# sfu-compbio/scalce

Hardware: AMD Instinct MI355X
Metric: input FASTQ MB/s compressed, 100 bp reads, bit-exact decompress (higher is better)
Workload: dtype u8

## Files before the change

scalce_amd/csrc/host_entropy.inc:

```
struct AcJob {
  scalce_batch *b;
  int m;
  const u8 *sym;
  u64 nsym;
  u32 nblk;
  bool general;
  u32 max_total = 0;
};
static const u64 AC_STRIDE = (u64)AC_BLOCK_SYMS + 4096;
constexpr u32 AC_LOG_WORDS = 1024;

static int ac_prepare(AcJob &j, hipStream_t s, bool framed_output = true, bool full_stride = false, bool allow_in_place = false) {
  scalce_batch *b = j.b;
  scalce_ctx *c = b->ctx;
  const int m = j.m;
  u32 *table = b->table[m].as<u32>();
  ENSURE(b, b->ac_tab[m], sizeof(uint4) * 512000);
  ENSURE(b, b->ac_cum[m], sizeof(u32) * 6400 * 81);
  BatchScratch::TableInfo *tinfo = &b->d_scr->tinfo[m];
  HIP_TRY(c, hipMemsetAsync(tinfo, 0, sizeof *tinfo, s));
  ENSURE(b, b->ac_tab8[m], sizeof(u64) * (6400 * 81 + 2));
  LAUNCH(ac_table_k, cdiv(6400, 64), 64, 0, s, table, b->ac_tab[m].as<uint4>(), b->ac_cum[m].as<u32>(), reinterpret_cast<u32 *>(&tinfo->max_total), b->ac_tab8[m].as<u64>(),
         tinfo->cost);
  BatchScratch::TableInfo th = {0, {0, 0}};
  { int rc = read_words(b, tinfo, &th, sizeof th / 4, s); if (rc) return rc; }
  const u32 max_total = (u32)th.max_total;
  j.general = max_total > (1u << 30) || getenv("SCALCE_AC_GENERAL") != nullptr;
  j.max_total = max_total;
  j.nblk = (u32)cdiv(j.nsym, AC_BLOCK_SYMS);
  {
    u64 stride = AC_STRIDE;
    const char *scale_env = getenv("SCALCE_AC_STRIDE_SCALE");
    const bool full = scale_env && atof(scale_env) == 0.0;
    if (!full && !full_stride && th.cost[1]) {
      double bytes_per_symbol = (double)th.cost[0] / 256.0 / 8.0 / (double)th.cost[1];
      if (scale_env) bytes_per_symbol *= atof(scale_env);
      const u64 est = (u64)((double)AC_BLOCK_SYMS * bytes_per_symbol * 1.08) + 65536;
      stride = std::min<u64>(AC_STRIDE, (est + 15) & ~15ull);
    }
    b->ac_stride[m] = stride;
  }
  b->in_place_now[m] = allow_in_place && b->code_in_place && !b->in_place_suspended && !b->qs_in_ws && j.nblk &&
                       j.sym == b->qs(m).as<u8>() && b->qs(m).cap >= j.nsym + 64 + AC_INPLACE_PAD;
  if (b->in_place_now[m]) {
    b->ac_stride[m] = AC_BLOCK_SYMS;
    b->ac_base[m] = b->qs(m).as<u8>();
    ENSURE(b, b->ac_log[m], sizeof(u32) * AC_LOG_WORDS * (size_t)j.nblk + 64);
  } else {
    ENSURE(b, b->ac_blocks[m], (size_t)j.nblk * b->ac_stride[m] + 4096 + 64);
    b->ac_base[m] = b->ac_blocks[m].as<u8>();
  }
  ENSURE(b, b->ac_sizes[m], sizeof(u32) * (j.nblk + 2));
  ENSURE(b, b->ac_off[m], sizeof(u64) * (j.nblk + 2));
  if (framed_output && !b->frame_on_demand) ENSURE(b, b->out_qual[m], (size_t)j.nblk * (b->ac_stride[m] + 4) + 64);
  ENSURE(b, b->ac_scan, sizeof(u64) * (scan_ws_elems(j.nblk ? j.nblk : 1) + 64));
  if (!j.nblk) b->out_qual_bytes[m] = 0;
  return SCALCE_OK;
}

enum AcLaunchKind { AC_SINGLE, AC_PAIRED, AC_RECODE, AC_WINDOW, AC_GROUP, AC_GROUP_LAST };
struct AcShape {
  int blocks_per_wg;
  u32 lanes;
};

static int ac_blocks_override() {
  const char *e = getenv("SCALCE_AC_BLOCKS_PER_WG");
  const int v = e ? atoi(e) : 0;
  return (v == 4 || v == 8 || v == 64) ? v : 0;
}

static u32 ac_lanes_override() {
  const char *e = getenv("SCALCE_AC_LANES_USED");
  if (!e) return 0;
  const int v = atoi(e);
  return (u32)(v < 1 || v > 64 ? 32 : v);
}

static AcShape ac_shape(AcLaunchKind kind, u32 blocks, bool general, int device) {
  const int over = ac_blocks_override();
  int bpw;
  switch (kind) {
    case AC_SINGLE: bpw = over ? over : 1; break;
    case AC_PAIRED:
    case AC_RECODE: bpw = blocks <= 1024 ? 4 : 8; break;
    case AC_WINDOW: bpw = 8; break;
    default:
      bpw = blocks < 900 ? 4 : (kind == AC_GROUP_LAST && blocks <= 2048) ? 8 : 64;
      if (over) bpw = over;
  }
  if (bpw == 64 && general) bpw = 8;
  u32 lanes = ac_lanes_override();
  if (!lanes && kind == AC_GROUP_LAST && bpw == 64) {
    static int n_cus = 0;
    if (!n_cus) { hipDeviceProp_t pr; n_cus = hipGetDeviceProperties(&pr, device) == hipSuccess && pr.multiProcessorCount > 0 ? pr.multiProcessorCount : 256; }
    lanes = std::min<u32>(std::max<u32>(cdiv(blocks, (u32)n_cus), 8u), 64u);
  }
  return AcShape{bpw, lanes ? lanes : 32u};
}

static int ac_launch(AcJob *jobs, int njobs, AcLaunchKind kind, hipStream_t s, hipStream_t ps) {
  scalce_batch *lead = jobs[0].b;
  scalce_ctx *c = lead->ctx;
  u32 total = 0;
  bool general = false;
  for (int i = 0; i < njobs; i++) {
    total += jobs[i].nblk;
    general |= jobs[i].general;
    if (jobs[i].max_total > (1u << 29)) general = true;
  }
  if (!total) return SCALCE_OK;
  const AcShape shape = ac_shape(kind, total, general, c->device);
  AcEncArgs a;
  memset(&a, 0, sizeof a);
  a.slow_threshold = 32;
  a.chain_prio = 3u;
  a.helper_prio = 0u;
  a.test_poison = getenv("SCALCE_AC_TEST_POISON") ? (u32)atoi(getenv("SCALCE_AC_TEST_POISON")) : 0u;
  a.inplace_shift = getenv("SCALCE_AC_INPLACE_TEST") ? 2u : 0u;
  a.simd_load = c->d_simd_load.as<u32>();
  if (const char *e = getenv("SCALCE_AC_SLOW_THRESHOLD")) a.slow_threshold = (u32)atoi(e);
  auto join = [&]() -> int {
    if (ps == s) return SCALCE_OK;
    hipEvent_t ev = lead->ev_group;
    if (!ev) { HIP_TRY(c, hipEventCreateWithFlags(&ev, hipEventDisableTiming)); lead->ev_group = ev; }
    HIP_TRY(c, hipEventRecord(ev, ps));
    HIP_TRY(c, hipStreamWaitEvent(s, ev, 0));
    return SCALCE_OK;
  };
  hipEvent_t ke0 = nullptr, ke1 = nullptr;
  if (lead->ktiming) {
    if (lead->kev_used == lead->kev.size()) {
      hipEvent_t x, y;
      HIP_TRY(c, hipEventCreate(&x));
      HIP_TRY(c, hipEventCreate(&y));
      lead->kev.emplace_back(x, y);
    }
    ke0 = lead->kev[lead->kev_used].first; ke1 = lead->kev[lead->kev_used].second;
    lead->kev_used++;
  }
  if (shape.blocks_per_wg == 1) {
    if (njobs != 1) { set_err(c, "internal: ac_encode_k takes one job"); return SCALCE_ERR_ARG; }
    scalce_batch *b = jobs[0].b;
    const int m = jobs[0].m;
    a.sym = jobs[0].sym; a.nsym = jobs[0].nsym; a.tab = b->ac_tab[m].as<uint4>(); a.out = b->ac_base[m];
    a.out_stride = b->ac_stride[m]; a.out_cap = (u32)b->ac_stride[m]; a.out_size = b->ac_sizes[m].as<u32>(); a.err = b->d_err;
    { int rc = join(); if (rc) return rc; }
    if (ke0) hipEventRecord(ke0, s);
    if (general) LAUNCH(ac_encode_k<true>, total, 128, 0, s, a);
    else LAUNCH(ac_encode_k<false>, total, 128, 0, s, a);
    if (ke1) hipEventRecord(ke1, s);
  } else {
    if (total > lead->ac_desc_cap) {
      if (lead->ac_desc_host) hipHostFree(lead->ac_desc_host);
      lead->ac_desc_host = nullptr;
      lead->ac_desc_cap = 0;
      const u32 cap = std::max<u32>(total + total / 2, 8192u);
      HIP_TRY(c, hipHostMalloc(reinterpret_cast<void **>(&lead->ac_desc_host), sizeof(AcBlockDesc) * (size_t)cap, hipHostMallocDefault));
      lead->ac_desc_cap = cap;
    }
    const bool lanes = shape.blocks_per_wg == 64;
    AcBlockDesc *d = lead->ac_desc_host;
    u32 nd = 0;
    for (int i = 0; i < njobs; i++) {
      scalce_batch *b = jobs[i].b;
      const int m = jobs[i].m;
      for (u32 k = 0; k < jobs[i].nblk; k++) {
        AcBlockDesc x;
        const u64 off = (u64)k * AC_BLOCK_SYMS;
        x.sym = jobs[i].sym + off;
        x.tab = lanes ? reinterpret_cast<const uint4 *>(b->ac_tab8[m].as<u64>()) : b->ac_tab[m].as<uint4>();
        x.dst = reinterpret_cast<u32 *>(b->ac_base[m] + (u64)k * b->ac_stride[m]);
        x.cap = (u32)b->ac_stride[m];
        x.flags = 0; x.log = nullptr; x.log_cap = 0; x.pad_ = 0;
        if (b->in_place_now[m]) {
          const u64 left = jobs[i].nsym - (u64)k * AC_BLOCK_SYMS;
          if (left < AC_BLOCK_SYMS) x.cap = (u32)std::min<u64>(AC_BLOCK_SYMS, (left + AC_INPLACE_PAD) & ~3ull);
          x.flags = AC_BLOCK_IN_PLACE;
          x.log = b->ac_log[m].as<u32>() + (size_t)k * AC_LOG_WORDS;
          x.log_cap = AC_LOG_WORDS;
        }
        x.out_size = b->ac_sizes[m].as<u32>() + k;
        x.err = b->d_err;
        x.n = (u32)std::min<u64>(AC_BLOCK_SYMS, jobs[i].nsym - off);
        x.index = k;
        d[nd++] = x;
      }
    }
    ENSURE(lead, lead->ac_desc, sizeof(AcBlockDesc) * (size_t)lead->ac_desc_cap);
    HIP_TRY(c, hipMemcpyAsync(lead->ac_desc.p, d, sizeof(AcBlockDesc) * total, hipMemcpyHostToDevice, ps));
    a.desc = lead->ac_desc.as<AcBlockDesc>();
    a.nblocks = total;
    a.out_cap = (u32)AC_STRIDE;
    { int rc = join(); if (rc) return rc; }
    if (ke0) hipEventRecord(ke0, s);
    if (lanes) {
      a.lanes_used = shape.lanes;
      if (a.lanes_used <= 48) LAUNCH((ac_encode_lanes_k<true, 1, 48, 5>), cdiv(total, a.lanes_used), 256, 0, s, a);
      else LAUNCH((ac_encode_lanes_k<true, 1, 64, 5>), cdiv(total, a.lanes_used), 256, 0, s, a);
    } else if (shape.blocks_per_wg == 8) {
      if (general) LAUNCH((ac_encode_rows_k<true, 8>), cdiv(total, 8), 320, 0, s, a);
      else LAUNCH((ac_encode_rows_k<false, 8>), cdiv(total, 8), 320, 0, s, a);
    } else {
      if (general) LAUNCH((ac_encode_rows_k<true, 16>), cdiv(total, 4), 192, 0, s, a);
      else LAUNCH((ac_encode_rows_k<false, 16>), cdiv(total, 4), 192, 0, s, a);
    }
    if (ke1) hipEventRecord(ke1, s);
  }
  for (int i = 0; i < njobs; i++) {
    lead->k_in_bytes += jobs[i].nsym;
    jobs[i].b->ac_last_sym[jobs[i].m] = jobs[i].sym;
    jobs[i].b->ac_last_nsym[jobs[i].m] = jobs[i].nsym;
  }
  return SCALCE_OK;
}

static int ac_frame(AcJob &j, hipStream_t s) {
  scalce_batch *b = j.b;
  const int m = j.m;
  b->frame_virtual[m] = 0;
  if (!j.nblk) return SCALCE_OK;
  exclusive_scan<u64>(AcFrameLen{b->ac_sizes[m].as<u32>()}, j.nblk, StoreTo<u64>{b->ac_off[m].as<u64>()}, b->ac_scan.as<u64>(),
                      &b->d_scr->frame_bytes[m], s);
  if (b->frame_on_demand) {
    b->frame_virtual[m] = j.nblk;
    b->ent_pending[m] = j.nblk;
    return SCALCE_OK;
  }
  if (b->out_qual[m].cap < (size_t)j.nblk * (b->ac_stride[m] + 4) + 64) {
    u64 total = 0;
    { int rc = read_u64(b, &b->d_scr->frame_bytes[m], &total, 1, s); if (rc) return rc; }
    if (b->out_qual[m].cap < total + 64) ENSURE(b, b->out_qual[m], (size_t)(total + total / 16) + (32u << 20));
  }
  LAUNCH(ac_frame_k, dim3(cdiv(b->ac_stride[m], 16 * 256), j.nblk), 256, 0, s, b->ac_base[m], b->ac_stride[m],
         b->ac_sizes[m].as<u32>(), b->ac_off[m].as<u64>(), b->out_qual[m].as<u8>());
  b->ent_pending[m] = j.nblk;
  return SCALCE_OK;
}

static int encode_stream(scalce_batch *b, int m, const u8 *d_sym, u64 nsym, hipStream_t s) {
  AcJob j{b, m, d_sym, nsym, 0, false};
  int rc = ac_prepare(j, s);
  if (rc) return rc;
  if ((rc = ac_launch(&j, 1, AC_SINGLE, s, s))) return rc;
  return ac_frame(j, s);
}

static int entropy_recode_full(scalce_batch *b, hipStream_t s) {
  std::vector<AcJob> jobs;
  for (int m = 0; m < b->nm; m++) {
    if (!b->ac_last_sym[m] || !b->ac_last_nsym[m]) continue;
    AcJob j{b, m, b->ac_last_sym[m], b->ac_last_nsym[m], 0, false};
    int rc = ac_prepare(j, s, false, true);
    if (rc) return rc;
    jobs.push_back(j);
  }
  if (jobs.empty()) return SCALCE_OK;
  int rc = ac_launch(jobs.data(), (int)jobs.size(), AC_RECODE, s, s);
  if (rc) return rc;
  for (auto &j : jobs) { b->frame_deferred[j.m] = j.nblk; b->ent_pending[j.m] = 0; }
  return SCALCE_OK;
}

static int entropy_rerun_from_text(scalce_batch *b, hipStream_t s) {
  scalce_ctx *c = b->ctx;
  if (b->appending || b->base != 0 || !b->piece_text[0] || (b->nm == 2 && !b->piece_text[1])) {
    set_err(c, "a block coded in place outgrew its input and the shard's text is not at hand to run it again (scalce_batch_set_code_in_place)");
    return SCALCE_ERR_CAPACITY;
  }
  static const bool dbg = getenv("SCALCE_TRACE") != nullptr;
  if (dbg) fprintf(stderr, "scalce: batch %p: a block coded in place caught up with its input: the shard is run again from its text\n", (void *)b);
  const u8 *t1 = b->piece_text[0], *t2 = b->ntext == 2 ? b->piece_text[1] : nullptr;
  const u64 n1 = b->text_bytes[0], n2 = b->ntext == 2 ? b->text_bytes[1] : 0;
  for (int m = 0; m < 2; m++) { b->frame_deferred[m] = 0; b->ent_pending[m] = 0; b->in_place_now[m] = false; }
  b->in_place_suspended = true;
  b->reruns++;
  int rc = scalce_batch_front(b, t1, n1, t2, n2, s);
  if (!rc) rc = scalce_batch_entropy(b, nullptr, s);
  b->in_place_suspended = false;
  return rc;
}

static int entropy_collect(scalce_batch *b, hipStream_t s) {
  {
    bool open = false, tight = false, in_place = false;
    for (int m = 0; m < b->nm; m++) {
      open |= b->frame_deferred[m] != 0 || b->ent_pending[m] != 0;
      tight |= b->ac_stride[m] != 0 && b->ac_stride[m] < AC_STRIDE;
      in_place |= b->in_place_now[m];
    }
    if (open && tight) {
      DevErr e;
      HIP_TRY(b->ctx, hipMemcpyAsync(&e, b->d_err, sizeof e, hipMemcpyDeviceToHost, s));
      HIP_TRY(b->ctx, hipStreamSynchronize(s));
      if (e.code == E_ACOVERFLOW) {
        if (getenv("SCALCE_TRACE"))
          fprintf(stderr, "scalce: batch %p: block %llu outgrew its %llu-byte buffer (it needed %u): coding the shard again at the full stride\n",
                  (void *)b, (unsigned long long)e.where, (unsigned long long)b->ac_stride[0], e.aux);
        HIP_TRY(b->ctx, hipMemsetAsync(b->d_err, 0, sizeof(DevErr), s));
        if (in_place) return entropy_rerun_from_text(b, s);
        int rc = entropy_recode_full(b, s);
        if (rc) return rc;
      }
    }
  }
  for (int m = 0; m < b->nm; m++) {
    if (b->frame_deferred[m]) {
      AcJob j{b, m, nullptr, 0, b->frame_deferred[m], false};
      b->frame_deferred[m] = 0;
      int rc = ac_frame(j, s);
      if (rc) return rc;
    }
    if (!b->ent_pending[m]) continue;
    u64 total = 0;
    if (b->frame_virtual[m]) {
      b->frame_off_host[m].resize(b->frame_virtual[m]);
      HIP_TRY(b->ctx, hipMemcpyAsync(b->frame_off_host[m].data(), b->ac_off[m].p, sizeof(u64) * b->frame_virtual[m], hipMemcpyDeviceToHost, s));
    }
    { int rc = read_u64(b, &b->d_scr->frame_bytes[m], &total, 1, s); if (rc) return rc; }
    b->out_qual_bytes[m] = total;
    b->k_out_bytes += total - 4ull * b->ent_pending[m];
    b->ent_pending[m] = 0;
  }
  return SCALCE_OK;
}

static int ac_table_for(scalce_batch *b, int m, const uint32_t *d_table_override, u64 nsym, hipStream_t s) {
  scalce_ctx *c = b->ctx;
  u32 *table = b->table[m].as<u32>();
  if (d_table_override) {
    HIP_TRY(c, hipMemcpyAsync(table, d_table_override + (size_t)m * 512000, sizeof(u32) * 512000, hipMemcpyDeviceToDevice, s));
  } else {
    const u32 factor = 1 + (u32)(nsym / 0xFFFFFFFFull);
    LAUNCH(ac_scale_k, cdiv(512000, 256), 256, 0, s, b->freq4[m].as<u64>(), factor, table);
  }
  return SCALCE_OK;
}

constexpr u32 AC_WINDOW_BLOCKS = 2048;
static int entropy_windowed(scalce_batch *b, const uint32_t *d_table_override, hipStream_t s) {
  scalce_ctx *c = b->ctx;
  const u64 N = b->N;
  u32 W = AC_WINDOW_BLOCKS / (u32)b->nm;
  if (const char *e = getenv("SCALCE_AC_WINDOW_BLOCKS")) W = (u32)std::max(1, atoi(e));
  u64 used[2] = {0, 0}, nsym[2] = {0, 0};
  u32 nblk[2] = {0, 0}, most = 0;
  for (int m = 0; m < b->nm; m++) {
    nsym[m] = N * (u64)b->L[m];
    nblk[m] = cdiv(nsym[m], AC_BLOCK_SYMS);
    most = nblk[m] > most ? nblk[m] : most;
    b->frame_virtual[m] = 0;
    b->frame_off_host[m].clear();
    int rc = ac_table_for(b, m, d_table_override, nsym[m], s);
    if (rc) return rc;
    b->out_qual_bytes[m] = 0;
  }
  bool first = true;
  for (u32 w0 = 0; w0 < most; w0 += W) {
    AcJob jobs[2];
    int nj = 0;
    for (int m = 0; m < b->nm; m++) {
      if (w0 >= nblk[m]) continue;
      const u64 off = (u64)w0 * AC_BLOCK_SYMS;
      const u64 n = std::min<u64>(nsym[m] - off, (u64)W * AC_BLOCK_SYMS);
      jobs[nj] = AcJob{b, m, b->qs(m).as<u8>() + off, n, 0, false};
      int rc = ac_prepare(jobs[nj], s, false, true);
      if (rc) return rc;
      nj++;
    }
    if (!nj) break;
    int rc = ac_launch(jobs, nj, AC_WINDOW, s, s);
    if (rc) return rc;
    for (int i = 0; i < nj; i++) {
      const int m = jobs[i].m;
      exclusive_scan<u64>(AcFrameLen{b->ac_sizes[m].as<u32>()}, jobs[i].nblk, StoreTo<u64>{b->ac_off[m].as<u64>()}, b->ac_scan.as<u64>(),
                          &b->d_scr->frame_bytes[m], s);
      u64 total = 0;
      if ((rc = read_u64(b, &b->d_scr->frame_bytes[m], &total, 1, s))) return rc;
      if (first) {
        const u64 est = (u64)((double)total / (double)jobs[i].nsym * 1.03 * (double)nsym[m]) + (64u << 20);
        ENSURE(b, b->out_qual[m], est);
      }
      if ((rc = ensure_keep(b, b->out_qual[m], used[m] + total + 64, used[m], s))) return rc;
      LAUNCH(ac_frame_k, dim3(cdiv(b->ac_stride[m], 16 * 256), jobs[i].nblk), 256, 0, s, b->ac_base[m], b->ac_stride[m],
             b->ac_sizes[m].as<u32>(), b->ac_off[m].as<u64>(), b->out_qual[m].as<u8>() + used[m]);
      used[m] += total;
      b->k_out_bytes += total - 4ull * jobs[i].nblk;
    }
    first = false;
  }
  HIP_TRY(c, hipStreamSynchronize(s));
  for (int m = 0; m < b->nm; m++) { b->out_qual_bytes[m] = used[m]; b->ent_pending[m] = 0; }
  return SCALCE_OK;
}

extern "C" int scalce_batch_entropy_begin(scalce_batch *b, const uint32_t *d_table_override, void *stream) {
  if (!b) return SCALCE_ERR_ARG;
  hipStream_t s = (hipStream_t)stream;
  scalce_ctx *c = b->ctx;
  HIP_TRY(c, hipSetDevice(c->device));
  if (b->nq) {
    for (int m = 0; m < b->nm; m++) b->out_qual_bytes[m] = 0;
    return SCALCE_OK;
  }
  const u64 N = b->N;
  if (!b->p.no_ac) {
    u64 blocks = 0;
    for (int m = 0; m < b->nm; m++) blocks += cdiv(N * (u64)b->L[m], AC_BLOCK_SYMS);
    if (blocks > AC_WINDOW_BLOCKS || getenv("SCALCE_AC_WINDOW_BLOCKS")) return entropy_windowed(b, d_table_override, s);
  }
  if (b->nm == 2 && !b->p.no_ac && !ac_blocks_override()) {
    AcJob jobs[2];
    for (int m = 0; m < 2; m++) {
      const u64 nsym = N * (u64)b->L[m];
      int rc = ac_table_for(b, m, d_table_override, nsym, s);
      if (rc) return rc;
      jobs[m] = AcJob{b, m, b->qs(m).as<u8>(), nsym, 0, false};
      if ((rc = ac_prepare(jobs[m], s))) return rc;
    }
    int rc = ac_launch(jobs, 2, AC_PAIRED, s, s);
    if (rc) return rc;
    for (int m = 0; m < 2; m++)
      if ((rc = ac_frame(jobs[m], s))) return rc;
    return SCALCE_OK;
  }
  for (int m = 0; m < b->nm; m++) {
    const u64 nsym = N * (u64)b->L[m];
    if (b->p.no_ac) {
      b->out_qual_bytes[m] = nsym;
      continue;
    }
    int rc = ac_table_for(b, m, d_table_override, nsym, s);
    if (rc) return rc;
    if ((rc = encode_stream(b, m, b->qs(m).as<u8>(), nsym, s))) return rc;
  }
  return SCALCE_OK;
}

extern "C" int scalce_batch_entropy_begin_group(scalce_batch **bs, int n, void *prep_stream, void *stream) {
  return scalce_batch_entropy_begin_group_last(bs, n, prep_stream, stream, 0);
}
extern "C" int scalce_batch_entropy_begin_group_last(scalce_batch **bs, int n, void *prep_stream, void *stream, int last) {
  if (!bs || n <= 0 || n > SCALCE_GROUP_MAX || (last != 0 && last != 1)) return SCALCE_ERR_ARG;
  for (int i = 0; i < n; i++) if (!bs[i] || bs[i]->ctx != bs[0]->ctx) return SCALCE_ERR_ARG;
  hipStream_t ps = (hipStream_t)prep_stream, s = (hipStream_t)stream;
  scalce_ctx *c = bs[0]->ctx;
  HIP_TRY(c, hipSetDevice(c->device));
  std::vector<AcJob> jobs;
  for (int i = 0; i < n; i++) {
    scalce_batch *b = bs[i];
    for (int m = 0; m < b->nm; m++) {
      const u64 own = b->N * (u64)b->L[m];
      if (b->nq) { b->out_qual_bytes[m] = 0; continue; }
      if (b->p.no_ac) { b->out_qual_bytes[m] = own; continue; }
      AcJob j{b, m, b->ent_external[m] ? b->ent_sym[m] : b->qs(m).as<u8>(), b->ent_external[m] ? b->ent_nsym[m] : own, 0, false};
      if (!b->ent_external[m]) { int rc = ac_table_for(b, m, nullptr, own, ps); if (rc) return rc; }
      b->ent_external[m] = false;
      int rc = ac_prepare(j, ps, false, false, true);
      if (rc) return rc;
      jobs.push_back(j);
    }
  }
  if (jobs.empty()) return SCALCE_OK;
  int rc = ac_launch(jobs.data(), (int)jobs.size(), last ? AC_GROUP_LAST : AC_GROUP, s, ps);
  if (rc) return rc;
  for (auto &j : jobs) j.b->frame_deferred[j.m] = j.nblk;
  return SCALCE_OK;
}

extern "C" int scalce_batch_entropy_stream_prepare(scalce_batch *b, int mate, const uint32_t *d_table, const uint8_t *d_symbols,
                                                   uint64_t nsym, void *stream) {
  if (!b || mate < 0 || mate >= b->nm || !d_table || (nsym && !d_symbols) || b->p.no_ac || b->nq) return SCALCE_ERR_ARG;
  scalce_ctx *c = b->ctx;
  HIP_TRY(c, hipSetDevice(c->device));
  HIP_TRY(c, hipMemcpyAsync(b->table[mate].p, d_table, sizeof(u32) * 512000, hipMemcpyDeviceToDevice, (hipStream_t)stream));
  b->ent_sym[mate] = d_symbols;
  b->ent_nsym[mate] = nsym;
  b->ent_external[mate] = true;
  return SCALCE_OK;
}

extern "C" int scalce_batch_entropy_end(scalce_batch *b, void *stream) {
  if (!b) return SCALCE_ERR_ARG;
  HIP_TRY(b->ctx, hipSetDevice(b->ctx->device));
  return entropy_collect(b, (hipStream_t)stream);
}

extern "C" int scalce_batch_entropy(scalce_batch *b, const uint32_t *d_table_override, void *stream) {
  if (!b) return SCALCE_ERR_ARG;
  if (b->nq) return scalce_batch_entropy_begin(b, d_table_override, stream);
  StageTimer tm(b, ST_ENTROPY, (hipStream_t)stream);
  int rc = scalce_batch_entropy_begin(b, d_table_override, stream);
  if (rc) return rc;
  return entropy_collect(b, (hipStream_t)stream);
}

extern "C" int scalce_batch_entropy_stream_begin(scalce_batch *b, int mate, const uint32_t *d_table, const uint8_t *d_symbols,
                                                 uint64_t nsym, void *stream) {
  if (!b || mate < 0 || mate >= b->nm || !d_table || (nsym && !d_symbols) || b->p.no_ac || b->nq) return SCALCE_ERR_ARG;
  hipStream_t s = (hipStream_t)stream;
  scalce_ctx *c = b->ctx;
  HIP_TRY(c, hipSetDevice(c->device));
  HIP_TRY(c, hipMemcpyAsync(b->table[mate].p, d_table, sizeof(u32) * 512000, hipMemcpyDeviceToDevice, s));
  return encode_stream(b, mate, d_symbols, nsym, s);
}
extern "C" int scalce_batch_entropy_stream(scalce_batch *b, int mate, const uint32_t *d_table, const uint8_t *d_symbols,
                                           uint64_t nsym, void *stream) {
  if (!b) return SCALCE_ERR_ARG;
  StageTimer tm(b, ST_ENTROPY, (hipStream_t)stream);
  int rc = scalce_batch_entropy_stream_begin(b, mate, d_table, d_symbols, nsym, stream);
  if (rc) return rc;
  return entropy_collect(b, (hipStream_t)stream);
}

extern "C" int scalce_ac_scale(scalce_ctx *c, const uint64_t *d_counters, uint32_t factor, uint32_t *d_table, void *stream) {
  if (!c || !d_counters || !d_table || !factor) return SCALCE_ERR_ARG;
  HIP_TRY(c, hipSetDevice(c->device));
  LAUNCH(ac_scale_k, cdiv(512000, 256), 256, 0, (hipStream_t)stream, reinterpret_cast<const u64 *>(d_counters), factor, d_table);
  return SCALCE_OK;
}

extern "C" int scalce_copy_pieces(scalce_ctx *c, const uint8_t *d_src, uint8_t *d_dst, const uint64_t *d_piece_src,
                                  const uint64_t *d_piece_dst, uint32_t npieces, uint64_t total_bytes, void *stream) {
  if (!c) return SCALCE_ERR_ARG;
  if (!npieces || !total_bytes) return SCALCE_OK;
  HIP_TRY(c, hipSetDevice(c->device));
  LAUNCH(copy_pieces_k, cdiv(total_bytes + 15, 256 * 16 * CP_CHUNKS), 256, 0, (hipStream_t)stream, d_src, d_dst,
         reinterpret_cast<const u64 *>(d_piece_src), reinterpret_cast<const u64 *>(d_piece_dst), npieces, (u64)total_bytes);
  return SCALCE_OK;
}
```

scalce_amd/csrc/kernels_acl.hpp:

```cpp
#pragma once
#include "kernels_ac.hpp"

namespace scalce {

constexpr int ACL_STEPS = 16;

__device__ __forceinline__ void acl_step_general(u32 &lo, u32 &hi, const uint4 g, u32 &B, u32 &t) {
  const u32 R = hi - lo;
  u32 M;
  const bool wrap = __builtin_add_overflow(R, 1u, &M);
  const u32 qa = mulfrac_m(M, wrap, g.z, g.w);
  const u32 qb = mulfrac_m(M, wrap, g.x, g.y);
  const u32 nhi = (g.w == 0xFFFFFFFFu) ? hi : lo + qa - 1;
  const u32 nlo = lo + qb;
  B = qb;
  const u32 x = nlo ^ nhi;
  const u32 kf = x ? (u32)__clz(x) : 31u;
  const u32 ks = kf < 31u ? kf : 31u;
  const u32 z = ((nlo & ~nhi) << ks) << 1;
  const u32 u = (u32)__clz(~z);
  t = ks + u;
  lo = (nlo << t) & 0x7FFFFFFFu;
  hi = (nhi << t) | ((1u << t) - 1) | 0x80000000u;
}

__device__ __forceinline__ void acl_step_plain(u32 &lo, u32 &M, const uint4 g, u32 ones, u32 zero, u32 &B, u32 &t) {
  const u32 A1 = (u32)(((u64)M * g.w + (((u64)ones << 32) | __umulhi(M, g.z))) >> 32);
  B = (u32)(((u64)M * g.y + (((u64)zero << 32) | __umulhi(M, g.x))) >> 32);
  const u32 D = A1 - B;
  const u32 nlo = lo + B;
  t = renorm_count(nlo, D);
  M = (D + 1) << t;
  lo = nlo << t;
}

template <int LW, int SETS> struct AclRing { static constexpr int WORDS = 64; };
template <int LW>
struct AclSink {
  SCALCE_GLOBAL u32 *dst;
  u32 wcap;
  SCALCE_GLOBAL u32 *logtop;
  u32 logcap;
  u32 w2, w1, w0;
  u32 Qb;
  u32 ncar;
  u32 nlog;
  bool over;
  __device__ __forceinline__ void init(SCALCE_GLOBAL u32 *d, u32 cap_words, SCALCE_GLOBAL u32 *log, u32 log_words, u32 s0, u32 s1) {
    dst = d; wcap = cap_words;
    logtop = log ? log + (log_words - 1u) : d + (cap_words - 1u);
    logcap = log ? log_words : 0u;
    w2 = 0; w1 = (s0 << 24) | (s1 << 16); w0 = 0;
    Qb = 16; ncar = ~0u; nlog = 0; over = false;
  }
  __device__ __forceinline__ u32 final_words() const {
    const u32 wq = Qb >> 5;
    return wq ? wq - 1u : 0u;
  }
  __device__ __forceinline__ bool room() {
    if ((Qb >> 5) + 2 * ACL_STEPS + 2 + (logcap ? 0u : nlog) >= wcap) over = true;
    if (logcap && nlog + ACL_STEPS + 2 >= logcap) over = true;
    return !over;
  }
  __device__ __forceinline__ void step(u32 B, u32 Qa, u32 &val, u32 &wq) {
    const u32 pos = Qb & 31u;
    const u32 b_hi = B >> pos;
    const u32 b_lo = __builtin_amdgcn_alignbit(B, 0u, pos);
    u32 c0, c1;
    w0 = __builtin_addc(w0, b_lo, 0u, &c0);
    w1 = __builtin_addc(w1, b_hi, c0, &c1);
    w2 += c1;
    ncar = w2 < ncar ? w2 : ncar;
    wq = Qb >> 5;
    val = w2;
    const bool f = (Qa >> 5) != wq;
    w2 = f ? w1 : w2;
    w1 = f ? w0 : w1;
    w0 = f ? 0u : w0;
    Qb = Qa;
  }
  __device__ __forceinline__ void careful(u32 B, u32 Qa) {
    const u32 pos = Qb & 31u;
    const u32 b_hi = B >> pos;
    const u32 b_lo = __builtin_amdgcn_alignbit(B, 0u, pos);
    u32 c0, c1, c2;
    w0 = __builtin_addc(w0, b_lo, 0u, &c0);
    w1 = __builtin_addc(w1, b_hi, c0, &c1);
    w2 = __builtin_addc(w2, 0u, c1, &c2);
    const u32 wq = Qb >> 5;
    if (c2 != 0u) {
      *(logtop - nlog) = wq - 2u;
      nlog++;
    }
    if ((Qa >> 5) != wq) { w2 = w1; w1 = w0; w0 = 0u; }
    Qb = Qa;
  }
  static __device__ __forceinline__ void carry_back(SCALCE_GLOBAL u32 *dst, u32 wcap, int k) {
    for (; k >= 0; k--) {
      if ((u32)k >= wcap) continue;
      const u32 v = __builtin_bswap32(__hip_atomic_load(&dst[k], __ATOMIC_RELAXED, __HIP_MEMORY_SCOPE_AGENT)) + 1u;
      __hip_atomic_store(&dst[k], __builtin_bswap32(v), __ATOMIC_RELAXED, __HIP_MEMORY_SCOPE_AGENT);
      if (v) break;
    }
  }
  __device__ __forceinline__ u32 finish(u32 final_lo) {
    const u32 pos = Qb & 31u;
    const int wi = (int)(Qb >> 5) - 1;
    const u64 ulp = 1ull << (62u - pos);
    u64 v = ((u64)w1 << 32) | w0;
    v = (v & ~(ulp - 1)) | ulp;
    if ((final_lo >> 30) & 1u) {
      const bool c = __builtin_add_overflow(v, ulp, &v);
      if (c) {
        w2 += 1u;
        if (w2 == 0u && !over) { *(logtop - nlog) = (u32)(wi - 1); nlog++; }
      }
    }
    const u32 bits = Qb + 2u;
    const u32 words[3] = {w2, (u32)(v >> 32), (u32)v};
#pragma unroll
    for (int k = 0; k < 3; k++) {
      const int idx = wi + k;
      if (idx >= 0 && 32u * (u32)idx < bits) {
        if ((u32)idx < wcap) dst[idx] = __builtin_bswap32(words[k]);
        else over = true;
      }
    }
    if (nlog && !over) {
      __threadfence();
      for (u32 e = 0; e < nlog; e++) {
        const int k = (int)__hip_atomic_load(logtop - e, __ATOMIC_RELAXED, __HIP_MEMORY_SCOPE_AGENT);
        carry_back(dst, wcap, k);
      }
    }
    return (bits + 7) >> 3;
  }
};

template <int LW, int SLOTS, int RINGW>
struct AclShared {
  uint4 ops[SLOTS][ACL_STEPS][LW];
  uint4 rec[2][ACL_STEPS / 2][LW];
  uint4 fifo[2][ACL_STEPS / 2][LW];
  u32 stage[RINGW][LW];
  u32 pub[2][LW];
  u32 final_lo[LW];
};

__device__ __forceinline__ u32x4 acl_load16(const SCALCE_GLOBAL u8 *p) {
  u32x4 v;
  asm volatile("global_load_dwordx4 %0, %1, off" : "=v"(v) : "v"(p) : "memory");
  return v;
}
template <int N>
__device__ __forceinline__ void acl_wait_vm(u32x4 &v) {
  asm volatile("s_waitcnt vmcnt(%1)" : "+v"(v) : "n"(N) : "memory");
}
template <int N>
__device__ __forceinline__ void acl_wait_vm() {
  asm volatile("s_waitcnt vmcnt(%0)" ::"n"(N) : "memory");
}

template <bool EXCLUSIVE, int SETS, int LW, int SLOTS>
__global__ __launch_bounds__(256 * SETS) void ac_encode_lanes_k(AcEncArgs a) {
  static_assert(SLOTS >= 3 && SLOTS <= 9 && LW <= 64 && (SETS == 1 || SETS == 2), "");
  __shared__ AclShared<LW, SLOTS, AclRing<LW, SETS>::WORDS> shs[SETS];
  const int lane = lane_id();
  const int w = wave_id();
  const u32 rtab = a.pairing == 1 ? 0x11332200u : a.pairing == 2 ? 0x33221100u : 0x33112200u;
  const u32 stab = a.pairing == 1 ? 0x01011010u : a.pairing == 2 ? 0x01011010u : 0x01011010u;
  const int role = SETS == 1 ? w : (int)((rtab >> (4 * w)) & 15u);
  const int set = SETS == 1 ? 0 : (int)((stab >> (4 * w)) & 15u);
  AclShared<LW, SLOTS, AclRing<LW, SETS>::WORDS> &sh = shs[set];
  const u32 nwg = gridDim.x, xq = nwg >> 3, xr = nwg & 7u, xcd = blockIdx.x & 7u;
  const u32 wg = (xcd < xr ? xcd * (xq + 1u) : xr * (xq + 1u) + (xcd - xr) * xq) + (blockIdx.x >> 3);
  const u32 bpw = a.lanes_used && a.lanes_used < (u32)LW ? a.lanes_used : (u32)LW;
  const u32 blk = (wg * SETS + (u32)set) * bpw + (u32)lane;
  const bool have = blk < a.nblocks && (u32)lane < bpw;
  const SCALCE_GLOBAL AcBlockDesc *dp = (const SCALCE_GLOBAL AcBlockDesc *)a.desc + (have ? blk : 0u);
  const u32 n = have ? dp->n : 0u;
  const u32 nr = (n + ACL_STEPS - 1) / ACL_STEPS;
  u32 nr_wg = nr;
  if (SETS == 2) {
    const u32 oblk = (wg * SETS + (u32)(set ^ 1)) * bpw + (u32)lane;
    const u32 on = oblk < a.nblocks && (u32)lane < bpw ? ((const SCALCE_GLOBAL AcBlockDesc *)a.desc + oblk)->n : 0u;
    const u32 onr = (on + ACL_STEPS - 1) / ACL_STEPS;
    nr_wg = onr > nr_wg ? onr : nr_wg;
  }
#pragma unroll
  for (int d = 32; d; d >>= 1) { const u32 o = __shfl_xor(nr_wg, d, 64); nr_wg = o > nr_wg ? o : nr_wg; }
  nr_wg = __builtin_amdgcn_readfirstlane(nr_wg);
  if (!nr_wg) return;
  if (EXCLUSIVE) {
    if (SETS == 1) asm volatile("" ::: "v255", "a255");
    else asm volatile("" ::: "v255");
  }
  if (SETS == 2 && (role & 1)) {
    if (a.helper_prio == 0) __builtin_amdgcn_s_setprio(0);
    else if (a.helper_prio == 1) __builtin_amdgcn_s_setprio(1);
    else if (a.helper_prio == 3) __builtin_amdgcn_s_setprio(3);
    else __builtin_amdgcn_s_setprio(2);
  } else __builtin_amdgcn_s_setprio(3);
  const bool inrow = LW == 64 || lane < LW;

  if (role == 1) {
    constexpr int AHEAD = SLOTS - 1;
    const SCALCE_GLOBAL u8 *sp = (const SCALCE_GLOBAL u8 *)dp->sym;
    const SCALCE_GLOBAL u64 *tab = (const SCALCE_GLOBAL u64 *)dp->tab;
    auto sym_addr = [&](u32 k) -> const SCALCE_GLOBAL u8 * {
      const u32 off = k * ACL_STEPS < n ? k * ACL_STEPS : 0u;
      return sp + off;
    };
    u32 p0 = 0, p1 = 0;
    auto request = [&](const u32x4 sy, u32 k) {
      uint4 *slot = &sh.ops[k % SLOTS][0][0];
#pragma unroll
      for (int j = 0; j < ACL_STEPS; j++) {
        const u32 word = j < 4 ? sy.x : j < 8 ? sy.y : j < 12 ? sy.z : sy.w;
        u32 c = (word >> (8 * (j & 3))) & 0xFFu;
        const u32 D1 = AC_D - 1;
        c = c < D1 ? c : D1;
        const u32 idx = (p0 * AC_D + p1) * (AC_D + 1) + c;
        __builtin_amdgcn_global_load_lds((const SCALCE_GLOBAL void *)(tab + idx), (__attribute__((address_space(3))) void *)(slot + j * LW), 16, 0, 0);
        p0 = p1;
        p1 = c;
      }
    };
    u32x4 ca[8], cb[8];
    auto load_chunk = [&](u32x4 (&c)[8], u32 first) {
#pragma unroll
      for (int q = 0; q < 8; q++) c[q] = acl_load16(sym_addr(first + q));
    };
    if (inrow) {
      load_chunk(ca, 0);
      load_chunk(cb, 8);
#pragma unroll
      for (int q = 0; q < 8; q++) { acl_wait_vm<0>(ca[q]); acl_wait_vm<0>(cb[q]); }
#pragma unroll
      for (int q = 0; q < AHEAD; q++) request(ca[q], q);
      acl_wait_vm<(AHEAD - 1) * 16>();
      asm volatile("s_barrier" ::: "memory");
      auto close = [&]() {
        acl_wait_vm<(AHEAD - 1) * 16>();
        asm volatile("s_barrier" ::: "memory");
      };
      for (u32 i0 = 0; i0 < nr_wg; i0 += 16) {
#pragma unroll
        for (int j = 0; j < 16; j++) {
          if (i0 + j < nr_wg) {
            const int e = (j + AHEAD) & 15;
            request(e < 8 ? ca[e] : cb[e - 8], i0 + j + AHEAD);
            if (j == 8 - AHEAD) load_chunk(ca, i0 + 16);
            if (j == 16 - AHEAD) load_chunk(cb, i0 + 24);
            close();
          }
        }
      }
      acl_wait_vm<0>();
      asm volatile("s_barrier" ::: "memory");
      asm volatile("s_barrier" ::: "memory");
    }
  } else if (role == 0) {
    u32 ones, zero;
    asm("v_mov_b32 %0, -1" : "=v"(ones));
    asm("v_mov_b32 %0, 0" : "=v"(zero));
    u32 lo = 0, M = 0;
    u32 Q = 16;
    if (inrow) {
      __syncthreads();
      for (u32 r = 0; r < nr_wg; r++) {
        const int slot = r % SLOTS;
        const u32 lo0 = lo, M0 = M, Q0 = Q;
        uint4 g[ACL_STEPS];
#pragma unroll
        for (int j = 0; j < ACL_STEPS; j++) g[j] = sh.ops[slot][j][lane];
        u32 topw = 0;
        u32 Bp = 0, Qp = 0;
#pragma unroll
        for (int j = 0; j < ACL_STEPS; j++) {
          u32 B, t;
          acl_step_plain(lo, M, g[j], ones, zero, B, t);
          Q += t;
          if (j & 1) sh.rec[r & 1][j >> 1][lane] = make_uint4(Qp, Bp, Q, B);
          else { Bp = B; Qp = Q; }
          topw = g[j].w > topw ? g[j].w : topw;
        }
        const bool live = r < nr;
        const bool poisoned = a.test_poison && r % a.test_poison == 0;
        const bool complete = r > 0 && r * ACL_STEPS + ACL_STEPS <= n;
        const bool fast_ok = complete && topw != 0xFFFFFFFFu && M0 != 0u && M != 0u && !poisoned;
        const bool fix = live && !fast_ok;
        if (__builtin_expect(__any(fix), 0)) {
          if (fix) {
            u32 glo = lo0 & 0x7FFFFFFFu, ghi = glo + M0 - 1u, gq = Q0;
            const u32 jstart = r == 0 ? 2u : 0u;
            const u32 left = n - r * ACL_STEPS;
            const u32 jend = left < (u32)ACL_STEPS ? left : (u32)ACL_STEPS;
            u32 Bp = 0, Qp = 0;
#pragma unroll 1
            for (u32 j = 0; j < (u32)ACL_STEPS; j++) {
              const uint4 gj = sh.ops[slot][j][lane];
              u32 B = 0, t = 0;
              if (j >= jstart && j < jend) acl_step_general(glo, ghi, gj, B, t);
              gq += t;
              if (j & 1u) sh.rec[r & 1][j >> 1][lane] = make_uint4(Qp, Bp, gq, B);
              else { Bp = B; Qp = gq; }
            }
            lo = glo;
            M = ghi - glo + 1u;
            Q = gq;
          }
        }
        if (r + 1 == nr) sh.final_lo[lane] = lo & 0x7FFFFFFFu;
        __syncthreads();
      }
      __syncthreads();
      __syncthreads();
    }
  } else if (role == 2) {
    if (inrow) {
      AclSink<LW> sk;
      {
        const SCALCE_GLOBAL u8 *sp = (const SCALCE_GLOBAL u8 *)dp->sym;
        const u32 s0 = n ? (u32)sp[0] : 0u, s1 = n > 1 ? (u32)sp[1] : 0u;
        sk.init((SCALCE_GLOBAL u32 *)dp->dst, dp->cap / 4, (SCALCE_GLOBAL u32 *)dp->log, dp->log_cap, s0, s1);
      }
      sh.pub[0][lane] = 0;
      sh.pub[1][lane] = 0;
      barrier_lds_only();
      auto take = [&](u32 r) {
        if (r < nr && sk.room()) {
          uint4 v[ACL_STEPS / 2];
#pragma unroll
          for (int j = 0; j < ACL_STEPS / 2; j++) v[j] = sh.rec[r & 1][j][lane];
          const u32 s2 = sk.w2, s1 = sk.w1, s0 = sk.w0, sq = sk.Qb;
          sk.ncar = ~0u;
#pragma unroll
          for (int j = 0; j < ACL_STEPS / 2; j++) {
            uint4 o;
            sk.step(v[j].y, v[j].x, o.x, o.y);
            sk.step(v[j].w, v[j].z, o.z, o.w);
            sh.fifo[r & 1][j][lane] = o;
          }
          if (__builtin_expect(__any(sk.ncar == 0u), 0)) {
            if (sk.ncar == 0u) {
              sk.w2 = s2; sk.w1 = s1; sk.w0 = s0; sk.Qb = sq;
#pragma unroll 1
              for (int j = 0; j < ACL_STEPS / 2; j++) {
                const uint4 x = sh.rec[r & 1][j][lane];
                sk.careful(x.y, x.x);
                sk.careful(x.w, x.z);
              }
            }
          }
        }
      };
      for (u32 i = 0; i < nr_wg; i++) {
        if (i > 0) take(i - 1);
        sh.pub[i & 1][lane] = sk.final_words();
        barrier_lds_only();
      }
      take(nr_wg - 1);
      sh.pub[nr_wg & 1][lane] = sk.final_words();
      barrier_lds_only();
      barrier_lds_only();
      if (have && n) {
        const u32 bytes = sk.finish(sh.final_lo[lane]);
        *(SCALCE_GLOBAL u32 *)dp->out_size = sk.over ? 0u : bytes;
        if (sk.over) dev_fail(dp->err, E_ACOVERFLOW, dp->index, bytes);
      }
    }
  } else {
    constexpr u32 RING = AclRing<LW, SETS>::WORDS;
    SCALCE_GLOBAL u32 *dst = (SCALCE_GLOBAL u32 *)dp->dst;
    const u32 wcap = dp->cap / 4;
    u32 wo = 0;
    const bool in_place = have && (dp->flags & AC_BLOCK_IN_PLACE) != 0;
    bool dead = false;
    auto word = [&](u32 k) -> u32 { return __builtin_bswap32(sh.stage[(k + 1u) & (RING - 1)][lane]); };
    auto drain = [&](u32 lim, u32 words_taken) {
      if (in_place && !dead && lim >= wo + 32u && wo + 32u > words_taken) {
        dead = true;
        dev_fail(dp->err, E_ACOVERFLOW, dp->index, 4u * (wo + 32u));
      }
      u64 ready = __ballot(inrow && !dead && lim >= wo + 32u);
      while (ready) {
        const u32 la = (u32)__builtin_ctzll(ready);
        ready &= ready - 1;
        const u32 lb = ready ? (u32)__builtin_ctzll(ready) : la;
        const bool two = ready != 0;
        ready &= ready - 1;
        const u32 t = (u32)lane & 31u;
        const bool up = lane >= 32;
        const u32 src = up ? lb : la;
        const u32 wo_a = (u32)__builtin_amdgcn_readlane(wo, la), wo_b = (u32)__builtin_amdgcn_readlane(wo, lb);
        const u32 cap_a = (u32)__builtin_amdgcn_readlane(wcap, la), cap_b = (u32)__builtin_amdgcn_readlane(wcap, lb);
        const u64 da = (u64)(uintptr_t)dst;
        const u32 dlo = (u32)da, dhi = (u32)(da >> 32);
        const u64 dst_a = ((u64)(u32)__builtin_amdgcn_readlane(dhi, la) << 32) | (u64)(u32)__builtin_amdgcn_readlane(dlo, la);
        const u64 dst_b = ((u64)(u32)__builtin_amdgcn_readlane(dhi, lb) << 32) | (u64)(u32)__builtin_amdgcn_readlane(dlo, lb);
        const u32 k = (up ? wo_b : wo_a) + t;
        const u32 v = __builtin_bswap32(sh.stage[(k + 1u) & (RING - 1)][src]);
        SCALCE_GLOBAL u32 *d = (SCALCE_GLOBAL u32 *)(uintptr_t)(up ? dst_b : dst_a);
        if ((!up || two) && k < (up ? cap_b : cap_a)) d[k] = v;
        if ((u32)lane == la || (two && (u32)lane == lb)) wo += 32;
      }
    };
    auto apply = [&](u32 r) {
      if (inrow && r < nr) {
        uint4 e[ACL_STEPS / 2];
#pragma unroll
        for (int j = 0; j < ACL_STEPS / 2; j++) e[j] = sh.fifo[r & 1][j][lane];
#pragma unroll
        for (int j = 0; j < ACL_STEPS / 2; j++) {
          sh.stage[e[j].y & (RING - 1)][lane] = e[j].x;
          sh.stage[e[j].w & (RING - 1)][lane] = e[j].z;
        }
      }
    };
    barrier_lds_only();
    for (u32 i = 0; i < nr_wg; i++) {
      if (i > 1) apply(i - 2);
      if (i > 0) drain(inrow ? sh.pub[(i - 1) & 1][lane] : 0u, i > 1 ? (4u * (i - 1u)) >> a.inplace_shift : 0u);
      barrier_lds_only();
    }
    barrier_lds_only();
    {
      if (nr_wg > 1) apply(nr_wg - 2);
      apply(nr_wg - 1);
      const u32 lim = inrow ? sh.pub[nr_wg & 1][lane] : 0u;
      drain(lim, ~0u);
      for (; wo < lim && !dead; wo++)
        if (wo < wcap) dst[wo] = word(wo);
      __threadfence();
    }
    barrier_lds_only();
  }
}

}
```

Measured before the change: 163,000.

## Deepen arithmetic-coder lane pipeline: extra slot, prefetched ops, early LDS reads

New measurement: 162,400. Within noise of the previous version (-0.4%).

```diff
diff --git a/scalce_amd/csrc/host_entropy.inc b/scalce_amd/csrc/host_entropy.inc
--- a/scalce_amd/csrc/host_entropy.inc
+++ b/scalce_amd/csrc/host_entropy.inc
@@ -196,8 +196,8 @@
     if (ke0) hipEventRecord(ke0, s);
     if (lanes) {
       a.lanes_used = shape.lanes;
-      if (a.lanes_used <= 48) LAUNCH((ac_encode_lanes_k<true, 1, 48, 5>), cdiv(total, a.lanes_used), 256, 0, s, a);
-      else LAUNCH((ac_encode_lanes_k<true, 1, 64, 5>), cdiv(total, a.lanes_used), 256, 0, s, a);
+      if (a.lanes_used <= 48) LAUNCH((ac_encode_lanes_k<true, 1, 48, 6>), cdiv(total, a.lanes_used), 256, 0, s, a);
+      else LAUNCH((ac_encode_lanes_k<true, 1, 64, 6>), cdiv(total, a.lanes_used), 256, 0, s, a);
     } else if (shape.blocks_per_wg == 8) {
       if (general) LAUNCH((ac_encode_rows_k<true, 8>), cdiv(total, 8), 320, 0, s, a);
       else LAUNCH((ac_encode_rows_k<false, 8>), cdiv(total, 8), 320, 0, s, a);
diff --git a/scalce_amd/csrc/kernels_acl.hpp b/scalce_amd/csrc/kernels_acl.hpp
--- a/scalce_amd/csrc/kernels_acl.hpp
+++ b/scalce_amd/csrc/kernels_acl.hpp
@@ -139,6 +139,7 @@
 
 template <int LW, int SLOTS, int RINGW>
 struct AclShared {
+  static_assert(SLOTS >= 3, "slots i and i + 1 belong to the chain wave, slot i - 1 to the gather wave's newest request");
   uint4 ops[SLOTS][ACL_STEPS][LW];
   uint4 rec[2][ACL_STEPS / 2][LW];
   uint4 fifo[2][ACL_STEPS / 2][LW];
@@ -159,6 +160,19 @@
 template <int N>
 __device__ __forceinline__ void acl_wait_vm() {
   asm volatile("s_waitcnt vmcnt(%0)" ::"n"(N) : "memory");
+}
+template <int OFFSET>
+__device__ __forceinline__ u32x4 acl_lds_read16(const uint4 *p) {
+  static_assert(OFFSET >= 0 && OFFSET < 65536, "");
+  u32x4 v;
+  asm volatile("ds_read_b128 %0, %1 offset:%2" : "=v"(v) : "v"((__attribute__((address_space(3))) const uint4 *)p), "n"(OFFSET) : "memory");
+  return v;
+}
+__device__ __forceinline__ void acl_wait_lds(u32x4 (&v)[ACL_STEPS / 2]) {
+  asm volatile("s_waitcnt lgkmcnt(0)"
+               : "+v"(v[0]), "+v"(v[1]), "+v"(v[2]), "+v"(v[3]), "+v"(v[4]), "+v"(v[5]), "+v"(v[6]), "+v"(v[7])
+               :
+               : "memory");
 }
 
 template <bool EXCLUSIVE, int SETS, int LW, int SLOTS>
@@ -238,10 +252,10 @@
       for (int q = 0; q < 8; q++) { acl_wait_vm<0>(ca[q]); acl_wait_vm<0>(cb[q]); }
 #pragma unroll
       for (int q = 0; q < AHEAD; q++) request(ca[q], q);
-      acl_wait_vm<(AHEAD - 1) * 16>();
+      acl_wait_vm<(AHEAD - 2) * 16>();
       asm volatile("s_barrier" ::: "memory");
       auto close = [&]() {
-        acl_wait_vm<(AHEAD - 1) * 16>();
+        acl_wait_vm<(AHEAD - 2) * 16>();
         asm volatile("s_barrier" ::: "memory");
       };
       for (u32 i0 = 0; i0 < nr_wg; i0 += 16) {
@@ -266,14 +280,16 @@
     asm("v_mov_b32 %0, 0" : "=v"(zero));
     u32 lo = 0, M = 0;
     u32 Q = 16;
+    u32 flo = 0;
     if (inrow) {
-      __syncthreads();
-      for (u32 r = 0; r < nr_wg; r++) {
-        const int slot = r % SLOTS;
+      barrier_lds_only();
+      auto fetch = [&](uint4 (&g)[ACL_STEPS], int slot) {
+#pragma unroll
+        for (int j = 0; j < ACL_STEPS; j++) g[j] = sh.ops[slot][j][lane];
+      };
+      auto round = [&](u32 r, int slot, const uint4 (&g)[ACL_STEPS], uint4 (&gn)[ACL_STEPS]) {
+        fetch(gn, slot + 1 == SLOTS ? 0 : slot + 1);
         const u32 lo0 = lo, M0 = M, Q0 = Q;
-        uint4 g[ACL_STEPS];
-#pragma unroll
-        for (int j = 0; j < ACL_STEPS; j++) g[j] = sh.ops[slot][j][lane];
         u32 topw = 0;
         u32 Bp = 0, Qp = 0;
 #pragma unroll
@@ -311,11 +327,22 @@
             Q = gq;
           }
         }
-        if (r + 1 == nr) sh.final_lo[lane] = lo & 0x7FFFFFFFu;
-        __syncthreads();
-      }
-      __syncthreads();
-      __syncthreads();
+        flo = r + 1 == nr ? lo : flo;
+        barrier_lds_only();
+      };
+      uint4 ga[ACL_STEPS], gb[ACL_STEPS];
+      fetch(ga, 0);
+      int slot = 0;
+      for (u32 r = 0; r < nr_wg; r += 2) {
+        round(r, slot, ga, gb);
+        slot = slot + 1 == SLOTS ? 0 : slot + 1;
+        if (r + 1 == nr_wg) break;
+        round(r + 1, slot, gb, ga);
+        slot = slot + 1 == SLOTS ? 0 : slot + 1;
+      }
+      sh.final_lo[lane] = flo & 0x7FFFFFFFu;
+      barrier_lds_only();
+      barrier_lds_only();
     }
   } else if (role == 2) {
     if (inrow) {
@@ -329,12 +356,18 @@
       sh.pub[1][lane] = 0;
       barrier_lds_only();
       auto take = [&](u32 r) {
+        u32x4 v[ACL_STEPS / 2];
+        {
+          const uint4 *p = &sh.rec[r & 1][0][lane];
+          constexpr int ROW = LW * 16;
+          v[0] = acl_lds_read16<0>(p);       v[1] = acl_lds_read16<ROW>(p);     v[2] = acl_lds_read16<2 * ROW>(p); v[3] = acl_lds_read16<3 * ROW>(p);
+          v[4] = acl_lds_read16<4 * ROW>(p); v[5] = acl_lds_read16<5 * ROW>(p); v[6] = acl_lds_read16<6 * ROW>(p); v[7] = acl_lds_read16<7 * ROW>(p);
+          static_assert(ACL_STEPS / 2 == 8, "");
+        }
         if (r < nr && sk.room()) {
-          uint4 v[ACL_STEPS / 2];
-#pragma unroll
-          for (int j = 0; j < ACL_STEPS / 2; j++) v[j] = sh.rec[r & 1][j][lane];
           const u32 s2 = sk.w2, s1 = sk.w1, s0 = sk.w0, sq = sk.Qb;
           sk.ncar = ~0u;
+          acl_wait_lds(v);
 #pragma unroll
           for (int j = 0; j < ACL_STEPS / 2; j++) {
             uint4 o;
@@ -354,6 +387,7 @@
             }
           }
         }
+        acl_wait_lds(v);
       };
       for (u32 i = 0; i < nr_wg; i++) {
         if (i > 0) take(i - 1);
```
